# GitHubOfAndrew/TeAMOFlow

Hardware: AMD Instinct MI355X
Metric: train_interactions_per_sec (higher is better)
Workload: dtype f32

## Files before the change

teamoflow_amd/csrc/tmf_common.h:

```cpp
#pragma once
#include <hip/hip_runtime.h>
#include <stdint.h>
#include <stdio.h>

#include <type_traits>

#include "../../include/tmf.h"

namespace tmf {

void set_error(const char* fmt, ...);
int check_launch(const char* what);

#define TMF_REQUIRE(cond, ...)             \
    do {                                   \
        if (!(cond)) {                     \
            tmf::set_error(__VA_ARGS__);   \
            return TMF_E_INVALID;          \
        }                                  \
    } while (0)

inline bool launch_fits(uint64_t blocks, unsigned threads) {
    return blocks > 0 && blocks < (1ull << 31) && blocks * threads < (1ull << 32);
}
// ... 300 lines not shown
    const tmf_f4 t = {v.x, v.y, v.z, v.w};
    __builtin_nontemporal_store(t, reinterpret_cast<tmf_f4*>(p));
}

template <int G, int NV>
__device__ __forceinline__ void store_row(const Frag<NV>& f, float* __restrict__ T, int64_t row, int g) {
    float* p = T + row * (int64_t)(4 * G * NV) + 4 * g;
#pragma unroll
    for (int v = 0; v < NV; ++v) store_f4_nt(p + 4 * G * v, f.v[v]);
}

template <int G, int NV>
__device__ __forceinline__ void store_row(const Frag<NV>& f, __bf16* __restrict__ T, int64_t row, int g) {
    bf16x8* p = reinterpret_cast<bf16x8*>(T + row * (int64_t)(4 * G * NV)) + g;
#pragma unroll
    for (int pv = 0; pv < NV / 2; ++pv) {
        f32x8 w;
        w[0] = f.v[2 * pv].x; w[1] = f.v[2 * pv].y; w[2] = f.v[2 * pv].z; w[3] = f.v[2 * pv].w;
        w[4] = f.v[2 * pv + 1].x; w[5] = f.v[2 * pv + 1].y; w[6] = f.v[2 * pv + 1].z; w[7] = f.v[2 * pv + 1].w;
        __builtin_nontemporal_store(__builtin_convertvector(w, bf16x8), p + G * pv);
    }
}

constexpr bool kNtFin = true;
template <int G, int NV, typename T, bool NT = false>
__device__ __forceinline__ void load_row_f32(Frag<NV>& f, const float* __restrict__ B, int64_t row, int g) {
    const float* p = B + row * (int64_t)(4 * G * NV);
#pragma unroll
    for (int v = 0; v < NV; ++v)
        f.v[v] = NT ? load_f4_nt(p + RowMap<G, NV, T>::off(v, g)) : *reinterpret_cast<const float4*>(p + RowMap<G, NV, T>::off(v, g));
}

template <int G, int NV, typename T>
__device__ __forceinline__ void store_row_f32(const Frag<NV>& f, float* __restrict__ B, int64_t row, int g) {
    float* p = B + row * (int64_t)(4 * G * NV);
#pragma unroll
    for (int v = 0; v < NV; ++v) store_f4_nt(p + RowMap<G, NV, T>::off(v, g), f.v[v]);
}

template <int NV>
__device__ __forceinline__ void zero(Frag<NV>& f) {
#pragma unroll
    for (int v = 0; v < NV; ++v) f.v[v] = make_float4(0.f, 0.f, 0.f, 0.f);
}

template <int NV>
__device__ __forceinline__ float dot_partial(const Frag<NV>& a, const Frag<NV>& b) {
    float s = 0.f;
#pragma unroll
    for (int v = 0; v < NV; ++v) {
        s = fmaf(a.v[v].x, b.v[v].x, s);
        s = fmaf(a.v[v].y, b.v[v].y, s);
        s = fmaf(a.v[v].z, b.v[v].z, s);
        s = fmaf(a.v[v].w, b.v[v].w, s);
    }
    return s;
}

template <int NV>
__device__ __forceinline__ void axpy(Frag<NV>& acc, float w, const Frag<NV>& x) {
#pragma unroll
    for (int v = 0; v < NV; ++v) {
        acc.v[v].x = fmaf(w, x.v[v].x, acc.v[v].x);
        acc.v[v].y = fmaf(w, x.v[v].y, acc.v[v].y);
        acc.v[v].z = fmaf(w, x.v[v].z, acc.v[v].z);
        acc.v[v].w = fmaf(w, x.v[v].w, acc.v[v].w);
    }
}

template <int NV>
__device__ __forceinline__ void add(Frag<NV>& acc, const Frag<NV>& x) {
#pragma unroll
    for (int v = 0; v < NV; ++v) {
        acc.v[v].x += x.v[v].x;
        acc.v[v].y += x.v[v].y;
        acc.v[v].z += x.v[v].z;
        acc.v[v].w += x.v[v].w;
    }
}

__device__ __forceinline__ void wave_lds_sync() {
    __builtin_amdgcn_fence(__ATOMIC_ACQ_REL, "wavefront");
    __builtin_amdgcn_wave_barrier();
}

template <int G>
__device__ __forceinline__ int group_read(int v, int idx) {
    return __shfl(v, (threadIdx.x & 63 & ~(G - 1)) + idx, 64);
}

constexpr int kSyncStride = 16;
__device__ __forceinline__ void step_rendezvous(int* sync, int i, int lag, int n_groups) {
    const int x = blockIdx.x & 7;
    const int mine = (n_groups - x + 7) / 8;
    __hip_atomic_fetch_add(sync + (i * 8 + x) * kSyncStride, 1, __ATOMIC_RELAXED, __HIP_MEMORY_SCOPE_AGENT);
    const int need = i - lag;
    if (need < 0) return;
    for (int spin = 0; spin < 256; ++spin) {
        if (__hip_atomic_load(sync + (need * 8 + x) * kSyncStride, __ATOMIC_RELAXED, __HIP_MEMORY_SCOPE_AGENT) >= mine) return;
        __builtin_amdgcn_s_sleep(8);
    }
}
inline size_t rendezvous_bytes(int64_t launches, int64_t steps) {
    return (size_t)launches * (size_t)steps * 8 * kSyncStride * sizeof(int);
}

#define TMF_DPP_ADD(v, ctrl) \
    ((v) + __int_as_float(__builtin_amdgcn_update_dpp(0, __float_as_int(v), (ctrl), 0xf, 0xf, false)))

template <int G>
__device__ __forceinline__ float group_allsum(float v) {
    if (G >= 2) v = TMF_DPP_ADD(v, 0xB1);
    if (G >= 4) v = TMF_DPP_ADD(v, 0x4E);
    if (G >= 8) v = TMF_DPP_ADD(v, 0x141);
    if (G >= 16) v = TMF_DPP_ADD(v, 0x140);
    if (G >= 32) {
        const auto r = __builtin_amdgcn_permlane16_swap(__float_as_int(v), __float_as_int(v), false, false);
        v = __int_as_float(r[0]) + __int_as_float(r[1]);
    }
    if (G >= 64) {
        const auto r = __builtin_amdgcn_permlane32_swap(__float_as_int(v), __float_as_int(v), false, false);
        v = __int_as_float(r[0]) + __int_as_float(r[1]);
    }
    return v;
}

template <int G>
__device__ __forceinline__ float across_groups_sum(float v) {
#pragma unroll
    for (int off = 32; off >= G; off >>= 1) v += __shfl_xor(v, off, 64);
    return v;
}

template <int G, int NV>
__device__ __forceinline__ void across_groups_sum(Frag<NV>& f) {
#pragma unroll
    for (int v = 0; v < NV; ++v) {
        f.v[v].x = across_groups_sum<G>(f.v[v].x);
        f.v[v].y = across_groups_sum<G>(f.v[v].y);
        f.v[v].z = across_groups_sum<G>(f.v[v].z);
        f.v[v].w = across_groups_sum<G>(f.v[v].w);
    }
}

__device__ __forceinline__ float adam_fresh(float w, float g, const tmf_adam a) {
    const float m = g * a.one_minus_b1;
    const float v = (g * g) * a.one_minus_b2;
    return w - __fdiv_rn(m * a.alpha, __fsqrt_rn(v) + a.eps);
}

template <int NV>
__device__ __forceinline__ void adam_fresh(Frag<NV>& w, const Frag<NV>& g, const tmf_adam a) {
#pragma unroll
    for (int v = 0; v < NV; ++v) {
        w.v[v].x = adam_fresh(w.v[v].x, g.v[v].x, a);
        w.v[v].y = adam_fresh(w.v[v].y, g.v[v].y, a);
        w.v[v].z = adam_fresh(w.v[v].z, g.v[v].z, a);
        w.v[v].w = adam_fresh(w.v[v].w, g.v[v].w, a);
    }
}

template <int G, int NV, typename T>
__device__ __forceinline__ void row_epilogue(const Frag<NV>& g, const T* __restrict__ X_old, void* __restrict__ X_out,
                                             int64_t row, int lane_in_group, int epi, const tmf_adam adam) {
    if (epi == TMF_EPI_GRAD) {
        store_row_f32<G, NV, T>(g, static_cast<float*>(X_out), row, lane_in_group);
// ... 94 lines not shown
```

teamoflow_amd/csrc/tmf_train.hip:

```cpp
#include <stdlib.h>
#include <type_traits>

#include "tmf_common.h"

namespace tmf {

constexpr int kWavesPerBlock = 2;
constexpr int kUnroll = 4;
constexpr int kMseUnroll = 4;
constexpr int64_t kMaxBlocks = ((int64_t)1 << 32) / (64 * kWavesPerBlock) - 1;

struct SegView {
    const int64_t* rowptr;
    const int32_t* seg_row;
    const int32_t* seg_chunk;
    const int32_t* seg_slab;
    int64_t nseg;
    int32_t chunk;
    int32_t row_mod;
    int64_t seg0;
    int xcd_run;
};

struct SegRange { int row; int64_t beg, end; };
// ... 119 lines not shown
                mom[2] += pos ? p : 0.0;
                mom[3] += neg ? p : 0.0;
                mom[4] += pos ? p * p : 0.0;
                mom[5] += neg ? p * p : 0.0;
            } else {
                const double w = pos ? a_pos + b_pos * (p - mu_pos) : a_neg + b_neg * (p - mu_neg);
                axpy<NV>(acc, (pos || neg) ? (float)w : 0.f, y);
            }
        }
    }
    if constexpr (MOMENTS) {
#pragma unroll
        for (int c = 0; c < kKlMoments; ++c) {
#pragma unroll
            for (int off = 32; off >= G; off >>= 1) mom[c] += __shfl_xor(mom[c], off, 64);
        }
        if (lane == 0) {
#pragma unroll
            for (int c = 0; c < kKlMoments; ++c) part[seg * kKlMoments + c] = mom[c];
        }
    } else {
        across_groups_sum<G, NV>(acc);
        if (grp == 0) finish_segment<G, NV, T>(sv, seg, acc, X_old, X_out, slab, row, g, epi, adam);
    }
}

__global__ __launch_bounds__(1024) void k_kl_coeffs(const double* __restrict__ part, int64_t nseg, double* __restrict__ loss_out,
                                                    double* __restrict__ coef) {
    __shared__ double sh[16][kKlMoments];
    const double2* p2 = reinterpret_cast<const double2*>(part);
    const int64_t n2 = 3 * nseg;
    double2 acc[3] = {make_double2(0.0, 0.0), make_double2(0.0, 0.0), make_double2(0.0, 0.0)};
    for (int64_t e0 = threadIdx.x; e0 < n2; e0 += 6 * 1024) {
        double2 v[6];
#pragma unroll
        for (int u = 0; u < 6; ++u) {
            const int64_t e = e0 + (int64_t)u * 1024;
            v[u] = (e < n2) ? p2[e] : make_double2(0.0, 0.0);
        }
#pragma unroll
        for (int u = 0; u < 6; ++u) {
            acc[u % 3].x += v[u].x;
            acc[u % 3].y += v[u].y;
        }
    }
    const int rot = threadIdx.x % 3;
    const double2 m0 = rot == 0 ? acc[0] : rot == 1 ? acc[2] : acc[1];
    const double2 m1 = rot == 0 ? acc[1] : rot == 1 ? acc[0] : acc[2];
    const double2 m2 = rot == 0 ? acc[2] : rot == 1 ? acc[1] : acc[0];
    double s[kKlMoments] = {m0.x, m0.y, m1.x, m1.y, m2.x, m2.y};
#pragma unroll
    for (int c = 0; c < kKlMoments; ++c) {
#pragma unroll
        for (int off = 32; off >= 1; off >>= 1) s[c] += __shfl_xor(s[c], off, 64);
    }
    if ((threadIdx.x & 63) == 0) {
#pragma unroll
        for (int c = 0; c < kKlMoments; ++c) sh[threadIdx.x >> 6][c] = s[c];
    }
    __syncthreads();
    if (threadIdx.x != 0) return;
    double t[kKlMoments];
#pragma unroll
    for (int c = 0; c < kKlMoments; ++c) {
        t[c] = sh[0][c];
        for (int w = 1; w < 16; ++w) t[c] += sh[w][c];
    }
    const double n_pos = t[0], n_neg = t[1];
    const double mu_pos = t[2] / n_pos, mu_neg = t[3] / n_neg;
    const double v_pos = t[4] / n_pos - mu_pos * mu_pos, v_neg = t[5] / n_neg - mu_neg * mu_neg;
    const double sigma = sqrt(v_pos + v_neg), d = mu_pos - mu_neg, z = d / sigma;
    const double phi = exp(-0.5 * z * z) * 0.3989422804014326779;
    loss_out[0] = 0.5 * erfc(z * 0.7071067811865475244);
    coef[0] = -phi / (sigma * n_pos);
    coef[1] = phi * d / (sigma * sigma * sigma * n_pos);
    coef[2] = mu_pos;
    coef[3] = phi / (sigma * n_neg);
    coef[4] = phi * d / (sigma * sigma * sigma * n_neg);
    coef[5] = mu_neg;
}

constexpr int kWsumTile = 512;
constexpr int kWsumUnroll = 4;

template <int G, int NV, typename T>
__global__ __launch_bounds__(64 * kWavesPerBlock) void k_wsum_pass(
    SegView sv, const int32_t* __restrict__ ent_row, const int32_t* __restrict__ ent_w,
    const float* __restrict__ wbuf, const T* __restrict__ Tab, const T* __restrict__ X_old,
    void* __restrict__ X_out, float* __restrict__ slab, int epi, tmf_adam adam) {
    constexpr int NG = 64 / G;
    __shared__ int s_ids[kWavesPerBlock][kWsumTile];
    __shared__ float s_w[kWavesPerBlock][kWsumTile];
    const int lane = threadIdx.x & 63, wave = threadIdx.x >> 6;
    const int64_t seg = sv.seg0 + (int64_t)blockIdx.x * kWavesPerBlock + wave;
    if (seg >= sv.nseg) return;
    const int g = lane & (G - 1), grp = lane / G;
    const int row = sv.seg_row[seg];
    const int64_t rbeg = sv.rowptr[row], rend = sv.rowptr[row + 1];
    const int64_t beg = rbeg + (int64_t)sv.seg_chunk[seg] * sv.chunk;
    const int64_t end = (beg + sv.chunk < rend) ? beg + sv.chunk : rend;
    int* ids = s_ids[wave];
    float* ws = s_w[wave];

    Frag<NV> acc;
    zero<NV>(acc);
    for (int64_t t0 = beg; t0 < end; t0 += kWsumTile) {
        const int cnt = (int)((end - t0 < kWsumTile) ? end - t0 : kWsumTile);
        for (int e = lane; e < cnt; e += 64) {
            ids[e] = ent_row[t0 + e];
            ws[e] = wbuf[ent_w[t0 + e]];
        }
        wave_lds_sync();
        for (int e0 = grp; e0 < cnt; e0 += NG * kUnroll) {
            Raw<NV, T> raw[kUnroll];
            float wc[kUnroll];
#pragma unroll
            for (int t = 0; t < kUnroll; ++t) {
                const int e = e0 + t * NG;
                wc[t] = (e < cnt) ? ws[e] : 0.f;
                if constexpr (std::is_same<T, float>::value) {
                    if (wc[t] != 0.f) load_raw<G, NV>(raw[t], Tab, ids[e], g);
                    else zero_raw<NV>(raw[t]);
                } else {
                    load_raw<G, NV>(raw[t], Tab, ids[wc[t] != 0.f ? e : 0], g);
                }
            }
#pragma unroll
            for (int t = 0; t < kUnroll; ++t) {
                Frag<NV> y;
                to_frag<NV>(y, raw[t]);
                axpy<NV>(acc, wc[t], y);
            }
        }
    }
    across_groups_sum<G, NV>(acc);
    if (grp == 0) finish_segment<G, NV, T>(sv, seg, acc, X_old, X_out, slab, row, g, epi, adam);
}

template <int G, int NV, typename T>
__global__ __launch_bounds__(64 * kWavesPerBlock) void k_wsum_pass_pg(
    SegView sv, const int32_t* __restrict__ ent_row, const int32_t* __restrict__ ent_w,
    const float* __restrict__ wbuf, const T* __restrict__ Tab, const T* __restrict__ X_old,
    void* __restrict__ X_out, float* __restrict__ slab, int epi, tmf_adam adam) {
    constexpr int NG = 64 / G, TILE = kWsumTile / NG;
    __shared__ __attribute__((aligned(16))) int s_ids[kWavesPerBlock][kWsumTile];
    __shared__ __attribute__((aligned(16))) float s_w[kWavesPerBlock][kWsumTile];
    const int lane = threadIdx.x & 63, wave = threadIdx.x >> 6;
    const int g = lane & (G - 1), grp = lane / G;
    int64_t blk = blockIdx.x;
    if (sv.xcd_run > 0) {
        const int64_t super = (int64_t)8 * sv.xcd_run, full = (int64_t)gridDim.x / super * super;
        if (blk < full) {
            const int64_t sc = blk / super, r = blk % super;
            blk = sc * super + (r & 7) * sv.xcd_run + (r >> 3);
        }
    }
    const int64_t seg = sv.seg0 + (blk * kWavesPerBlock + wave) * NG + grp;
    const bool live = seg < sv.nseg;
    const int row = live ? sv.seg_row[seg] : 0;
    int64_t beg = 0, end = 0;
    if (live) {
        const int64_t rbeg = sv.rowptr[row], rend = sv.rowptr[row + 1];
        beg = rbeg + (int64_t)sv.seg_chunk[seg] * sv.chunk;
        end = (beg + sv.chunk < rend) ? beg + sv.chunk : rend;
    }
    int* ids = s_ids[wave] + grp * TILE;
    float* ws = s_w[wave] + grp * TILE;
    Frag<NV> acc;
    zero<NV>(acc);
    for (int64_t t0 = beg; t0 < end; t0 += TILE) {
        const int cnt = (int)((end - t0 < TILE) ? end - t0 : TILE);
        for (int e = g; e < cnt; e += G) {
            ids[e] = ent_row[t0 + e];
            ws[e] = wbuf[ent_w[t0 + e]];
        }
        wave_lds_sync();
        for (int e0 = 0; e0 < cnt; e0 += kWsumUnroll) {
            Raw<NV, T> raw[kWsumUnroll];
            float wc[kWsumUnroll];
#pragma unroll
            for (int t = 0; t < kWsumUnroll; ++t) {
                const int e = e0 + t;
                wc[t] = (e < cnt) ? ws[e] : 0.f;
                if constexpr (std::is_same<T, float>::value) {
                    if (wc[t] != 0.f) load_raw<G, NV>(raw[t], Tab, ids[e], g);
                    else zero_raw<NV>(raw[t]);
                } else {
                    load_raw<G, NV>(raw[t], Tab, ids[wc[t] != 0.f ? e : 0], g);
                }
            }
#pragma unroll
            for (int t = 0; t < kWsumUnroll; ++t) {
                Frag<NV> y;
                to_frag<NV>(y, raw[t]);
                axpy<NV>(acc, wc[t], y);
            }
        }
    }
    if (live) finish_segment<G, NV, T>(sv, seg, acc, X_old, X_out, slab, row, g, epi, adam);
}

constexpr int kRows4Tile = 64;
constexpr int kRows4Unroll2 = 6, kRows4Unroll1 = 4;
constexpr int kRows4Waves = 8;
constexpr int kRows4MinWaves = kRows4Waves / 2;
constexpr int kRows4K2 = 6;

struct VRows {
    const int32_t* item;
    const int32_t* part;
    const int32_t* nparts;
    const int32_t* slot;
    float* slab;
};

template <int G, int NV, typename T, int K, int WAVES>
__global__ __launch_bounds__(64 * WAVES, kRows4MinWaves) void k_wsum_rows4(
    const int64_t* __restrict__ rowptr, int64_t n_rows, int n_blocks, const int32_t* __restrict__ ent_row,
    const int32_t* __restrict__ ent_w, const float* __restrict__ wbuf, const T* __restrict__ Tab, const T* __restrict__ X_old,
    void* __restrict__ X_out, int epi, tmf_adam adam, int64_t row_begin, int64_t row_end, int* __restrict__ sync, int lag,
    VRows vr) {
    static_assert(K + 1 <= G, "the list boundaries of a block live in one register of the lane group");
    constexpr int NG = 64 / G, NGB = NG * WAVES, U = NV >= 2 ? kRows4Unroll2 : kRows4Unroll1;
    __shared__ int s_ids[NGB][kRows4Tile];
    __shared__ float s_w[NGB][kRows4Tile];
    const int tid = threadIdx.x, lane = tid & 63, wave = tid >> 6;
    const int g = lane & (G - 1), gid = wave * NG + lane / G;
    int* ids = s_ids[gid];
    float* ws = s_w[gid];
    const int64_t j0 = row_begin + ((int64_t)blockIdx.x * NGB + gid) * K;
    const int kv = (int)((row_end - j0 < K) ? (row_end > j0 ? row_end - j0 : 0) : K);
    Frag<NV> acc[K];
#pragma unroll
    for (int k = 0; k < K; ++k) zero<NV>(acc[k]);
    const bool balanced = vr.item != nullptr;
    const int64_t vq = j0 + (g < kv ? g : kv);
    const int64_t it = (balanced && kv > 0) ? (int64_t)vr.item[vq] : vq;
    const int pt = (balanced && kv > 0) ? vr.part[vq] : 0, np = (balanced && kv > 0) ? vr.nparts[vq] : 1;
    for (int t = 0; t < n_blocks; ++t) {
        int bnd = 0;
        if (kv > 0) {
            const int64_t lb = rowptr[(int64_t)t * n_rows + it];
            bnd = (int)lb;
            if (np > 1) bnd += (int)(((int64_t)pt * (rowptr[(int64_t)t * n_rows + it + 1] - lb)) / np);
        }
        const int r_beg = group_read<G>(bnd, 0), r_end = group_read<G>(bnd, kv);
        int b[K + 1];
#pragma unroll
        for (int k = 0; k <= K; ++k) b[k] = group_read<G>(bnd, k < kv ? k : kv);
        for (int c0 = r_beg; c0 < r_end; c0 += kRows4Tile) {
            const int cnt = (r_end - c0 < kRows4Tile) ? r_end - c0 : kRows4Tile;
            for (int e = g; e < cnt; e += G) {
                ids[e] = ent_row[c0 + e];
                ws[e] = wbuf[ent_w[c0 + e]];
            }
            wave_lds_sync();
#pragma unroll
            for (int k = 0; k < K; ++k) {
                const int lo = (b[k] > c0 ? b[k] : c0) - c0;
                const int hi = ((b[k + 1] < c0 + cnt) ? b[k + 1] : c0 + cnt) - c0;
                for (int e0 = lo; e0 < hi; e0 += U) {
                    Raw<NV, T> raw[U];
                    float wc[U];
#pragma unroll
                    for (int u = 0; u < U; ++u) {
                        const int e = e0 + u;
                        wc[u] = (e < hi) ? ws[e] : 0.f;
                        load_raw<G, NV>(raw[u], Tab, ids[(wc[u] != 0.f) ? e : lo], g);
                    }
#pragma unroll
                    for (int u = 0; u < U; ++u) {
                        Frag<NV> y;
// ... 461 lines not shown
```

teamoflow_amd/csrc/tmf_wmrb.hip:

```cpp
#include <math.h>
#include <stdlib.h>

#include <type_traits>

#include "tmf_common.h"

namespace tmf {

constexpr int kThreads = 256;
constexpr int kWaves = kThreads / 64;
constexpr int kPosChunk = 512;
constexpr int kUnrollW = 4;
constexpr int kG4Unroll = 4;

__host__ __device__ inline int round4(int x) { return (x + 3) & ~3; }

__host__ __device__ inline int sp_padded(int S) {
    const int nf4 = (S + 3) / 4;
    const int per = ((nf4 + 2 * kWaves - 1) / (2 * kWaves) + 1) & ~1;
    return 4 * 2 * kWaves * per;
}

__device__ __forceinline__ void count_ge0_x4(int& c0, int& c1, float x0, float x1, float x2, float x3) {
    unsigned long long m0, m1, m2, m3;
// ... 230 lines not shown

    across_groups_sum<G, NV>(acc);
#pragma unroll
    for (int off = 32; off >= 1; off >>= 1) {
        lsum += __shfl_xor(lsum, off, 64);
        npos += __shfl_xor(npos, off, 64);
    }
    __syncthreads();
    if (grp == 0) {
#pragma unroll
        for (int v = 0; v < NV; ++v) reinterpret_cast<float4*>(red + wave * LD)[g + G * v] = acc.v[v];
    }
    if (lane == 0) {
        red[kWaves * LD + wave] = lsum;
        red[kWaves * LD + kWaves + wave] = npos;
    }
    __syncthreads();
    if (wave == 0 && grp == 0) {
        Frag<NV> tot;
#pragma unroll
        for (int v = 0; v < NV; ++v) tot.v[v] = reinterpret_cast<const float4*>(red)[g + G * v];
        for (int w = 1; w < kWaves; ++w) {
            Frag<NV> part;
#pragma unroll
            for (int v = 0; v < NV; ++v) part.v[v] = reinterpret_cast<const float4*>(red + w * LD)[g + G * v];
            add<NV>(tot, part);
        }
        row_epilogue<G, NV, T>(tot, U_old, U_out, u, g, epi, adam);
    }
    if (tid == 0) {
        const float* t = red + kWaves * LD;
        if (loss_part) loss_part[u] = (t[0] + t[1]) + (t[2] + t[3]);
        if (pos_part) pos_part[u] = (t[4] + t[5]) + (t[6] + t[7]);
    }
}

template <int G, int NV, typename T>
__global__ __launch_bounds__(kThreads) void k_wmrb_user(
    const int64_t* __restrict__ rowptr, const int32_t* __restrict__ col, const float* __restrict__ val,
    const int32_t* __restrict__ R, int S, float c,
    const T* __restrict__ U_old, const T* __restrict__ V_old, void* __restrict__ U_out, float* __restrict__ delta,
    float* __restrict__ Dg, float* __restrict__ loss_part, float* __restrict__ pos_part, int epi, tmf_adam adam) {
    extern __shared__ __attribute__((aligned(16))) char smem_raw[];
    wmrb_user_body<G, NV, T>(blockIdx.x, smem_raw, rowptr, col, val, R, S, c, U_old, V_old, U_out, delta, Dg, loss_part,
                             pos_part, epi, adam);
}

static size_t wmrb_user_lds(int S, int ld) {
    return sizeof(float) * ((size_t)sp_padded(S) + round4(S) + 4 * kPosChunk + (size_t)round4(S) + 2 * kWaves * 64 +
                            (size_t)kWaves * ld + 2 * kWaves);
}

template <int G, int NV, typename T>
static int launch_wmrb_user(const int64_t* rowptr, const int32_t* col, const float* val, const int32_t* R,
                            int32_t n_users, int32_t S, float c, const T* U_old, const T* V_old,
                            void* U_out, float* delta, float* D, float* loss_part, float* pos_part, int epi,
                            tmf_adam adam, hipStream_t stream) {
    const size_t lds = wmrb_user_lds(S, 4 * G * NV);
    if (lds > 160 * 1024) {
        set_error("wmrb_user_pass: n_samples=%d does not fit LDS (%zu bytes); use the sliced pass (tmf_wmrb_scores3 ...)", S, lds);
        return TMF_E_UNSUPPORTED;
    }
    static LdsGrant grant;
    if (int rc = grant_dynamic_lds(reinterpret_cast<const void*>(&k_wmrb_user<G, NV, T>), lds, grant)) return rc;
    TMF_REQUIRE_LAUNCH(n_users, kThreads, "wmrb_user_pass");
    hipLaunchKernelGGL((k_wmrb_user<G, NV, T>), dim3((unsigned)n_users), dim3(kThreads), lds, stream, rowptr, col,
                       val, R, (int)S, c, U_old, V_old, U_out, delta, D, loss_part, pos_part, epi, adam);
    return check_launch("tmf_wmrb_user_pass");
}

constexpr int kSliceUsers = 16;
constexpr int kLongRange = 48;

template <int G>
struct Stage {
    static constexpr int tile = 8 * G;
};

template <int G>
__device__ __forceinline__ int* slice_stage(char* smem_raw, int gid) {
    return reinterpret_cast<int*>(smem_raw) + gid * 2 * Stage<G>::tile;
}

template <int G, int NV, typename T, bool GRADU>
__device__ __forceinline__ void slice_list(int* ids, float* dst, const int32_t* __restrict__ list, int beg, int end,
                                           const T* __restrict__ V, const Frag<NV>& x, Frag<NV>& acc,
                                           float* __restrict__ out, const float* __restrict__ wts, int g, int safe) {
    constexpr int kStageTile = Stage<G>::tile;
    for (int t0 = beg; t0 < end; t0 += kStageTile) {
        const int cnt = (end - t0 < kStageTile) ? end - t0 : kStageTile;
        for (int e = g; e < cnt; e += G) {
            ids[e] = __builtin_nontemporal_load(list + t0 + e);
            if (GRADU) dst[e] = __builtin_nontemporal_load(wts + t0 + e);
        }
        wave_lds_sync();
        float keep = 0.f;
        for (int e0 = 0; e0 < cnt; e0 += kUnrollW) {
            Raw<NV, T> raw[kUnrollW];
            float d[kUnrollW];
            static_assert(kUnrollW == 4, "vector LDS reads assume four entries per step");
            const int4 id4 = *reinterpret_cast<const int4*>(ids + e0);
            const float4 w4 = GRADU ? *reinterpret_cast<const float4*>(dst + e0) : make_float4(0.f, 0.f, 0.f, 0.f);
            const int idv[4] = {id4.x, id4.y, id4.z, id4.w};
            const float wv[4] = {w4.x, w4.y, w4.z, w4.w};
#pragma unroll
            for (int t = 0; t < kUnrollW; ++t) {
                const int e = e0 + t;
                bool want = e < cnt;
                d[t] = 0.f;
                if (GRADU && want) { d[t] = wv[t]; want = d[t] != 0.f; }
                load_raw<G, NV>(raw[t], V, want ? idv[t] : safe, g);
            }
#pragma unroll
            for (int t = 0; t < kUnrollW; ++t) {
                Frag<NV> y;
                to_frag<NV>(y, raw[t]);
                if (GRADU) {
                    axpy<NV>(acc, d[t], y);
                } else {
                    const int e = e0 + t;
                    const float pr = group_allsum<G>(dot_partial<NV>(x, y));
                    if (g == (e & (G - 1))) keep = pr;
                    if (e < cnt && ((e & (G - 1)) == G - 1 || e == cnt - 1)) {
                        if (g <= (e & (G - 1))) __builtin_nontemporal_store(keep, out + t0 + (e & ~(G - 1)) + g);
                    }
                }
            }
        }
    }
}

template <int NV, typename T>
__device__ __forceinline__ void slice_scores_lean(int* ids, const int32_t* __restrict__ list, int beg, int end, const T* __restrict__ V,
                                                  const Raw<NV, T>& x, float* __restrict__ out, int g, int lane, int safe) {
    constexpr int G = 32, kStageTile = Stage<G>::tile;
    const uint32_t loff = 16u * (uint32_t)g;
    const int my_entry = Reduce4x32::entry_of_lane(lane);
    const int my_step = lane & 7, my_slot = 4 * my_step + my_entry;
    for (int t0 = beg; t0 < end; t0 += kStageTile) {
        const int cnt = (end - t0 < kStageTile) ? end - t0 : kStageTile;
        const int cnt4 = (cnt + 3) & ~3;
        for (int e = g; e < cnt4; e += G) ids[e] = e < cnt ? __builtin_nontemporal_load(list + t0 + e) : safe;
        wave_lds_sync();
        float keep = 0.f;
        for (int e0 = 0; e0 < cnt4; e0 += 4) {
            const int4 id4 = *reinterpret_cast<const int4*>(ids + e0);
            Raw<NV, T> y[4];
            load_raw32<G, NV>(y[0], V, (uint32_t)id4.x, loff);
            load_raw32<G, NV>(y[1], V, (uint32_t)id4.y, loff);
            load_raw32<G, NV>(y[2], V, (uint32_t)id4.z, loff);
            load_raw32<G, NV>(y[3], V, (uint32_t)id4.w, loff);
            float pr[4];
#pragma unroll
            for (int t = 0; t < 4; ++t) pr[t] = dot_raw<NV>(x, y[t]);
            const float sc = Reduce4x32::run(pr, lane);
            const int step = (e0 >> 2) & 7;
            keep = (step == my_step) ? sc : keep;
            if (step == 7 || e0 + 4 >= cnt4) {
                const int at = (e0 & ~31) + my_slot;
                if (at < cnt) __builtin_nontemporal_store(keep, out + t0 + at);
            }
        }
    }
}

struct SliceLists {
    const int32_t* R;
    const int32_t* off;
    const int64_t* rowptr;
    const int32_t* col;
    const int32_t* poff;
    int n_slices, S;
    int64_t n_users, n_groups;
    int upg;
    int sl0, nsl;
    int item_base;
    int xcd;
    int lean;
};

__device__ __forceinline__ bool slice_of_block(const SliceLists& a, int64_t b, int64_t& sl, int64_t& grp) {
    if (!a.xcd) {
        sl = a.sl0 + b / a.n_groups;
        grp = b % a.n_groups;
        return true;
    }
    const int64_t x = b & 7, j = b >> 3;
    sl = a.sl0 + 8 * (j / a.n_groups) + x;
    grp = j % a.n_groups;
    return sl < a.sl0 + a.nsl;
}

template <int G, int NV, typename T>
__device__ __forceinline__ const T* window_base(const T* V, int item_base) {
    return V - (int64_t)item_base * (4 * G * NV);
}

template <int G, int NV, typename T, int WAVES>
__global__ __launch_bounds__(64 * WAVES) void k_wmrb_scores3(SliceLists a, const T* __restrict__ U, const T* __restrict__ V,
                                                           float* __restrict__ sp, float* __restrict__ p) {
    extern __shared__ __attribute__((aligned(16))) char smem_raw[];
    constexpr int NG = 64 / G, NGB = NG * WAVES;
    const int tid = threadIdx.x, lane = tid & 63, wave = tid >> 6;
    const int g = lane & (G - 1), gid = wave * NG + lane / G;
    int* ids = slice_stage<G>(smem_raw, gid);
    float* dst = reinterpret_cast<float*>(ids + Stage<G>::tile);
    int64_t sl, grp;
    if (!slice_of_block(a, blockIdx.x, sl, grp)) return;
    const int64_t ubeg = grp * a.upg;
    const int64_t uend = (ubeg + a.upg < a.n_users) ? ubeg + a.upg : a.n_users;
    V = window_base<G, NV, T>(V, a.item_base);
    if constexpr (G == 32 && sizeof(Raw<NV, T>) <= 16) {
        if (a.lean) {
            for (int64_t u = ubeg + gid; u < uend; u += NGB) {
                const int64_t o = u * (a.n_slices + 1) + sl;
                const int nb = a.off[o], ne = a.off[o + 1], pb = a.poff[o], pe = a.poff[o + 1];
                if (nb == ne && pb == pe) continue;
                Raw<NV, T> x;
                {
                    const char* xp = reinterpret_cast<const char*>(U) + u * (int64_t)RowBytes<G, NV, T>::value + 16 * g;
                    if constexpr (std::is_same<T, float>::value) {
#pragma unroll
                        for (int v = 0; v < NV; ++v) x.v[v] = load_f4_nt(reinterpret_cast<const float*>(xp + 16 * G * v));
                    } else {
#pragma unroll
                        for (int pv = 0; pv < NV / 2; ++pv) x.v[pv] = __builtin_nontemporal_load(reinterpret_cast<const bf16x8*>(xp + 16 * G * pv));
                    }
                }
                slice_scores_lean<NV, T>(ids, a.R + u * (int64_t)a.S, nb, ne, V, x, sp + u * (int64_t)a.S, g, lane, a.item_base);
                const int64_t rb = a.rowptr[u];
                slice_scores_lean<NV, T>(ids, a.col + rb, pb, pe, V, x, p + rb, g, lane, a.item_base);
            }
            return;
        }
    }
    for (int64_t u = ubeg + gid; u < uend; u += NGB) {
        const int64_t o = u * (a.n_slices + 1) + sl;
        const int nb = a.off[o], ne = a.off[o + 1], pb = a.poff[o], pe = a.poff[o + 1];
        if (nb == ne && pb == pe) continue;
        Frag<NV> x, none;
        load_row_nt<G, NV>(x, U, u, g);
        slice_list<G, NV, T, false>(ids, dst, a.R + u * (int64_t)a.S, nb, ne, V, x, none, sp + u * (int64_t)a.S, nullptr, g,
                                    a.item_base);
        const int64_t rb = a.rowptr[u];
        slice_list<G, NV, T, false>(ids, dst, a.col + rb, pb, pe, V, x, none, p + rb, nullptr, g, a.item_base);
    }
}

template <int G, int NV, typename T, int WAVES>
__global__ __launch_bounds__(64 * WAVES) void k_wmrb_gradu3(SliceLists a, const T* __restrict__ V, const float* __restrict__ D,
                                                          const float* __restrict__ delta, float* __restrict__ part,
                                                          int slice_first, int accumulate) {
    extern __shared__ __attribute__((aligned(16))) char smem_raw[];
    constexpr int NG = 64 / G, NGB = NG * WAVES;
    const int tid = threadIdx.x, lane = tid & 63, wave = tid >> 6;
    const int g = lane & (G - 1), gid = wave * NG + lane / G;
    int* ids = slice_stage<G>(smem_raw, gid);
    float* dst = reinterpret_cast<float*>(ids + Stage<G>::tile);
    int64_t sl, grp, layer = 0;
    if (slice_first < 0) {
        if (!slice_of_block(a, blockIdx.x, sl, grp)) return;
    } else if (accumulate >= 3) {
        layer = blockIdx.x & 7;
        sl = slice_first + layer;
        grp = blockIdx.x >> 3;
        if (sl >= a.sl0 + a.nsl) return;
        accumulate -= 2;
    } else {
        sl = slice_first;
        grp = blockIdx.x;
    }
    V = window_base<G, NV, T>(V, a.item_base);
    const int64_t ubeg = grp * a.upg;
    const int64_t uend = (ubeg + a.upg < a.n_users) ? ubeg + a.upg : a.n_users;
    for (int64_t u = ubeg + gid; u < uend; u += NGB) {
        const int64_t o = u * (a.n_slices + 1) + sl;
        const int nb = a.off[o], ne = a.off[o + 1], pb = a.poff[o], pe = a.poff[o + 1];
        Frag<NV> acc, none;
        zero<NV>(acc);
        const int64_t us = u * (int64_t)a.S, rb = a.rowptr[u];
        slice_list<G, NV, T, true>(ids, dst, a.R + us, nb, ne, V, none, acc, nullptr, D + us, g, a.item_base);
        slice_list<G, NV, T, true>(ids, dst, a.col + rb, pb, pe, V, none, acc, nullptr, delta + rb, g, a.item_base);
        if (accumulate == 0) {
            store_row_f32<G, NV, T>(acc, part, sl * a.n_users + u, g);
        } else {
            const int64_t prow = layer * a.n_users + u;
            if (accumulate == 2) {
                Frag<NV> prev;
                load_row_f32<G, NV, T>(prev, part, prow, g);
                add<NV>(prev, acc);
                acc = prev;
            }
            store_row_f32<G, NV, T>(acc, part, prow, g);
        }
    }
}

template <int G>
struct Stage4 {
    static constexpr int cap = G < 16 ? G : 16;
};

template <int G, int NV, typename T, int K, int WAVES>
__global__ __launch_bounds__(64 * WAVES, WAVES / 2) void k_wmrb_gradu4(
    SliceLists a, const T* __restrict__ V, const float* __restrict__ D,
                                                          const float* __restrict__ delta, const T* __restrict__ U_old,
                                                          void* __restrict__ U_out, int epi, tmf_adam adam, int64_t user_begin,
                                                          int64_t user_end, int* __restrict__ sync, int lag) {
    extern __shared__ __attribute__((aligned(16))) char smem_raw[];
    constexpr int NG = 64 / G, NGB = NG * WAVES, CAP = Stage4<G>::cap, WIN = G - 1, UG = (CAP >= 8) ? kG4Unroll : kUnrollW;
    const int tid = threadIdx.x, lane = tid & 63, wave = tid >> 6;
    const int g = lane & (G - 1), gid = wave * NG + lane / G;
    int* stage = reinterpret_cast<int*>(smem_raw) + gid * (2 * K * 2 * CAP);
    V = window_base<G, NV, T>(V, a.item_base);
    const int64_t u0 = user_begin + ((int64_t)blockIdx.x * NGB + gid) * K;
    const int sl_end = a.sl0 + a.nsl;
    Frag<NV> acc[K];
    int us[K], rb[K];
    bool live[K];
    int ocn[K], ocp[K];
    int c_tot[K];
#pragma unroll
    for (int k = 0; k < K; ++k) {
        zero<NV>(acc[k]);
        live[k] = u0 + k < user_end;
        const int64_t u = live[k] ? u0 + k : user_begin;
        us[k] = (int)(u * (int64_t)a.S);
        rb[k] = (int)a.rowptr[u];
    }
    int base = a.sl0;
    auto refill = [&](int b) {
        base = b;
#pragma unroll
        for (int k = 0; k < K; ++k) {
            const int64_t u = live[k] ? u0 + k : user_begin;
            const int64_t o = u * (a.n_slices + 1) + ((b + g <= a.n_slices) ? b + g : a.n_slices);
            ocn[k] = a.off[o];
            ocp[k] = a.poff[o];
        }
    };
    int n_tot[K], n_id[K];
    float n_w[K];
    auto fetch = [&](int sl) {
#pragma unroll
        for (int k = 0; k < K; ++k) {
            const int nb = group_read<G>(ocn[k], sl - base), ne = group_read<G>(ocn[k], sl + 1 - base);
            const int pb = group_read<G>(ocp[k], sl - base), pe = group_read<G>(ocp[k], sl + 1 - base);
            const int cn = live[k] ? ne - nb : 0;
            n_tot[k] = live[k] ? cn + (pe - pb) : 0;
            const bool neg = g < cn, any = g < n_tot[k] && g < CAP;
            const int at = neg ? us[k] + nb + g : rb[k] + pb + (g - cn);
            n_id[k] = any ? (neg ? a.R : a.col)[at] : a.item_base;
            n_w[k] = any ? (neg ? D : delta)[at] : 0.f;
        }
    };
    auto commit = [&](int buf) {
#pragma unroll
        for (int k = 0; k < K; ++k) {
            int* ids = stage + (buf * K + k) * 2 * CAP;
            if (g < CAP) {
                ids[g] = n_id[k];
                reinterpret_cast<float*>(ids + CAP)[g] = n_w[k];
            }
            c_tot[k] = n_tot[k];
        }
// ... 766 lines not shown
```

Before: 1.148 billion.

## Compact nonzero-weight entries via ballot before gathering embedding rows

```diff
diff --git a/teamoflow_amd/csrc/tmf_common.h b/teamoflow_amd/csrc/tmf_common.h
--- a/teamoflow_amd/csrc/tmf_common.h
+++ b/teamoflow_amd/csrc/tmf_common.h
@@ -406,6 +406,33 @@
 __device__ __forceinline__ void wave_lds_sync() {
     __builtin_amdgcn_fence(__ATOMIC_ACQ_REL, "wavefront");
     __builtin_amdgcn_wave_barrier();
+}
+
+template <int G, int STEP>
+__device__ __forceinline__ void stage_nonzero(int* ids, float* ws, int& n, int id, float w, int g) {
+    const bool nz = w != 0.f;
+    uint64_t b = __builtin_amdgcn_ballot_w64(nz);
+    if constexpr (G < 64) b = (b >> (threadIdx.x & 63 & ~(G - 1))) & ((1ull << G) - 1);
+    if (nz) {
+        const int at = n + __popcll(b & ((1ull << g) - 1));
+        ids[at] = id;
+        ws[at] = w;
+        if ((b >> g) == 1) {
+#pragma unroll
+            for (int k = 1; k < STEP; ++k) {
+                if ((at & (STEP - 1)) + k < STEP) {
+                    ids[at + k] = id;
+                    ws[at + k] = 0.f;
+                }
+            }
+        }
+    }
+    n += __popcll(b);
+}
+
+template <int STEP>
+__device__ __forceinline__ int staged_steps(int n) {
+    return (n + STEP - 1) / STEP * STEP;
 }
 
 template <int G>
diff --git a/teamoflow_amd/csrc/tmf_train.hip b/teamoflow_amd/csrc/tmf_train.hip
--- a/teamoflow_amd/csrc/tmf_train.hip
+++ b/teamoflow_amd/csrc/tmf_train.hip
@@ -225,6 +225,7 @@
 
 constexpr int kWsumTile = 512;
 constexpr int kWsumUnroll = 4;
+constexpr int kWsumRounds = 4;
 
 template <int G, int NV, typename T>
 __global__ __launch_bounds__(64 * kWavesPerBlock) void k_wsum_pass(
@@ -245,28 +246,54 @@
     int* ids = s_ids[wave];
     float* ws = s_w[wave];
 
+    constexpr int SUB = kWsumTile / NG;
+    constexpr uint64_t kClass0 = NG == 64 ? 1ull : ~0ull / ((1ull << (NG & 63)) - 1);
+    static_assert(SUB % kUnroll == 0, "a class's slots hold its padded count");
+    const int cls = lane & (NG - 1);
+    const uint64_t in_cls = kClass0 << cls, in_grp = kClass0 << grp, below = (1ull << lane) - 1;
     Frag<NV> acc;
     zero<NV>(acc);
     for (int64_t t0 = beg; t0 < end; t0 += kWsumTile) {
         const int cnt = (int)((end - t0 < kWsumTile) ? end - t0 : kWsumTile);
-        for (int e = lane; e < cnt; e += 64) {
-            ids[e] = ent_row[t0 + e];
-            ws[e] = wbuf[ent_w[t0 + e]];
-        }
+        int n_cls = 0, n = 0;
+        for (int e0 = 0; e0 < cnt; e0 += 64) {
+            const int e = e0 + lane;
+            int id = 0;
+            float w = 0.f;
+            if (e < cnt) {
+                id = ent_row[t0 + e];
+                w = wbuf[ent_w[t0 + e]];
+            }
+            const bool nz = w != 0.f;
+            const uint64_t b = __builtin_amdgcn_ballot_w64(nz);
+            if (nz) {
+                const int at = cls * SUB + n_cls + __popcll(b & in_cls & below);
+                ids[at] = id;
+                ws[at] = w;
+                if (((b & in_cls) >> lane) == 1) {
+#pragma unroll
+                    for (int k = 1; k < kUnroll; ++k) {
+                        if ((at & (kUnroll - 1)) + k < kUnroll) {
+                            ids[at + k] = id;
+                            ws[at + k] = 0.f;
+                        }
+                    }
+                }
+            }
+            n_cls += __popcll(b & in_cls);
+            n += __popcll(b & in_grp);
+        }
+        const int* idg = ids + grp * SUB;
+        const float* wsg = ws + grp * SUB;
+        n = staged_steps<kUnroll>(n);
         wave_lds_sync();
-        for (int e0 = grp; e0 < cnt; e0 += NG * kUnroll) {
+        for (int e0 = 0; e0 < n; e0 += kUnroll) {
             Raw<NV, T> raw[kUnroll];
             float wc[kUnroll];
 #pragma unroll
             for (int t = 0; t < kUnroll; ++t) {
-                const int e = e0 + t * NG;
-                wc[t] = (e < cnt) ? ws[e] : 0.f;
-                if constexpr (std::is_same<T, float>::value) {
-                    if (wc[t] != 0.f) load_raw<G, NV>(raw[t], Tab, ids[e], g);
-                    else zero_raw<NV>(raw[t]);
-                } else {
-                    load_raw<G, NV>(raw[t], Tab, ids[wc[t] != 0.f ? e : 0], g);
-                }
+                wc[t] = wsg[e0 + t];
+                load_raw<G, NV>(raw[t], Tab, idg[e0 + t], g);
             }
 #pragma unroll
             for (int t = 0; t < kUnroll; ++t) {
@@ -311,26 +338,36 @@
     float* ws = s_w[wave] + grp * TILE;
     Frag<NV> acc;
     zero<NV>(acc);
+    static_assert(TILE % kWsumUnroll == 0, "the tile buffers hold the padded count");
     for (int64_t t0 = beg; t0 < end; t0 += TILE) {
         const int cnt = (int)((end - t0 < TILE) ? end - t0 : TILE);
-        for (int e = g; e < cnt; e += G) {
-            ids[e] = ent_row[t0 + e];
-            ws[e] = wbuf[ent_w[t0 + e]];
-        }
+        int n = 0;
+        for (int e0 = 0; e0 < cnt; e0 += kWsumRounds * G) {
+            int id[kWsumRounds], iw[kWsumRounds];
+            float w[kWsumRounds];
+#pragma unroll
+            for (int k = 0; k < kWsumRounds; ++k) {
+                const int e = e0 + k * G + g;
+                id[k] = iw[k] = -1;
+                if (e < cnt) {
+                    id[k] = ent_row[t0 + e];
+                    iw[k] = ent_w[t0 + e];
+                }
+            }
+#pragma unroll
+            for (int k = 0; k < kWsumRounds; ++k) w[k] = iw[k] >= 0 ? wbuf[iw[k]] : 0.f;
+#pragma unroll
+            for (int k = 0; k < kWsumRounds; ++k) stage_nonzero<G, kWsumUnroll>(ids, ws, n, id[k], w[k], g);
+        }
+        n = staged_steps<kWsumUnroll>(n);
         wave_lds_sync();
-        for (int e0 = 0; e0 < cnt; e0 += kWsumUnroll) {
+        for (int e0 = 0; e0 < n; e0 += kWsumUnroll) {
             Raw<NV, T> raw[kWsumUnroll];
             float wc[kWsumUnroll];
 #pragma unroll
             for (int t = 0; t < kWsumUnroll; ++t) {
-                const int e = e0 + t;
-                wc[t] = (e < cnt) ? ws[e] : 0.f;
-                if constexpr (std::is_same<T, float>::value) {
-                    if (wc[t] != 0.f) load_raw<G, NV>(raw[t], Tab, ids[e], g);
-                    else zero_raw<NV>(raw[t]);
-                } else {
-                    load_raw<G, NV>(raw[t], Tab, ids[wc[t] != 0.f ? e : 0], g);
-                }
+                wc[t] = ws[e0 + t];
+                load_raw<G, NV>(raw[t], Tab, ids[e0 + t], g);
             }
 #pragma unroll
             for (int t = 0; t < kWsumUnroll; ++t) {
diff --git a/teamoflow_amd/csrc/tmf_wmrb.hip b/teamoflow_amd/csrc/tmf_wmrb.hip
--- a/teamoflow_amd/csrc/tmf_wmrb.hip
+++ b/teamoflow_amd/csrc/tmf_wmrb.hip
@@ -336,51 +336,86 @@
     return reinterpret_cast<int*>(smem_raw) + gid * 2 * Stage<G>::tile;
 }
 
-template <int G, int NV, typename T, bool GRADU>
-__device__ __forceinline__ void slice_list(int* ids, float* dst, const int32_t* __restrict__ list, int beg, int end,
-                                           const T* __restrict__ V, const Frag<NV>& x, Frag<NV>& acc,
-                                           float* __restrict__ out, const float* __restrict__ wts, int g, int safe) {
+template <int G, int NV, typename T>
+__device__ __forceinline__ void slice_list(int* ids, const int32_t* __restrict__ list, int beg, int end, const T* __restrict__ V,
+                                           const Frag<NV>& x, float* __restrict__ out, int g, int safe) {
     constexpr int kStageTile = Stage<G>::tile;
+    static_assert(kUnrollW == 4, "vector LDS reads assume four entries per step");
     for (int t0 = beg; t0 < end; t0 += kStageTile) {
         const int cnt = (end - t0 < kStageTile) ? end - t0 : kStageTile;
-        for (int e = g; e < cnt; e += G) {
-            ids[e] = __builtin_nontemporal_load(list + t0 + e);
-            if (GRADU) dst[e] = __builtin_nontemporal_load(wts + t0 + e);
-        }
+        for (int e = g; e < cnt; e += G) ids[e] = __builtin_nontemporal_load(list + t0 + e);
         wave_lds_sync();
         float keep = 0.f;
         for (int e0 = 0; e0 < cnt; e0 += kUnrollW) {
             Raw<NV, T> raw[kUnrollW];
-            float d[kUnrollW];
-            static_assert(kUnrollW == 4, "vector LDS reads assume four entries per step");
             const int4 id4 = *reinterpret_cast<const int4*>(ids + e0);
-            const float4 w4 = GRADU ? *reinterpret_cast<const float4*>(dst + e0) : make_float4(0.f, 0.f, 0.f, 0.f);
             const int idv[4] = {id4.x, id4.y, id4.z, id4.w};
-            const float wv[4] = {w4.x, w4.y, w4.z, w4.w};
-#pragma unroll
-            for (int t = 0; t < kUnrollW; ++t) {
-                const int e = e0 + t;
-                bool want = e < cnt;
-                d[t] = 0.f;
-                if (GRADU && want) { d[t] = wv[t]; want = d[t] != 0.f; }
-                load_raw<G, NV>(raw[t], V, want ? idv[t] : safe, g);
-            }
+#pragma unroll
+            for (int t = 0; t < kUnrollW; ++t)
+                load_raw<G, NV>(raw[t], V, e0 + t < cnt ? idv[t] : safe, g);
 #pragma unroll
             for (int t = 0; t < kUnrollW; ++t) {
                 Frag<NV> y;
                 to_frag<NV>(y, raw[t]);
-                if (GRADU) {
-                    axpy<NV>(acc, d[t], y);
-                } else {
-                    const int e = e0 + t;
-                    const float pr = group_allsum<G>(dot_partial<NV>(x, y));
-                    if (g == (e & (G - 1))) keep = pr;
-                    if (e < cnt && ((e & (G - 1)) == G - 1 || e == cnt - 1)) {
-                        if (g <= (e & (G - 1))) __builtin_nontemporal_store(keep, out + t0 + (e & ~(G - 1)) + g);
-                    }
+                const int e = e0 + t;
+                const float pr = group_allsum<G>(dot_partial<NV>(x, y));
+                if (g == (e & (G - 1))) keep = pr;
+                if (e < cnt && ((e & (G - 1)) == G - 1 || e == cnt - 1)) {
+                    if (g <= (e & (G - 1))) __builtin_nontemporal_store(keep, out + t0 + (e & ~(G - 1)) + g);
                 }
             }
         }
+    }
+}
+
+constexpr int kStageRounds = 4;
+
+template <int G, int NV, typename T>
+__device__ __forceinline__ void gather_staged(const int* ids, const float* ws, int n, const T* __restrict__ V, Frag<NV>& acc, int g) {
+    static_assert(kUnrollW == 4, "vector LDS reads assume four entries per step");
+    wave_lds_sync();
+    for (int e0 = 0; e0 < n; e0 += kUnrollW) {
+        Raw<NV, T> raw[kUnrollW];
+        const int4 id4 = *reinterpret_cast<const int4*>(ids + e0);
+        const float4 w4 = *reinterpret_cast<const float4*>(ws + e0);
+        const int idv[4] = {id4.x, id4.y, id4.z, id4.w};
+        const float wv[4] = {w4.x, w4.y, w4.z, w4.w};
+#pragma unroll
+        for (int t = 0; t < kUnrollW; ++t) load_raw<G, NV>(raw[t], V, idv[t], g);
+#pragma unroll
+        for (int t = 0; t < kUnrollW; ++t) {
+            Frag<NV> y;
+            to_frag<NV>(y, raw[t]);
+            axpy<NV>(acc, wv[t], y);
+        }
+    }
+}
+
+template <int G, int NV, typename T>
+__device__ __forceinline__ void slice_append(int* ids, float* ws, int& n, const int32_t* __restrict__ list,
+                                            const float* __restrict__ wts, int beg, int end, const T* __restrict__ V,
+                                            Frag<NV>& acc, int g) {
+    constexpr int kStageTile = Stage<G>::tile;
+    static_assert(kStageRounds * 2 <= 8, "a tile of 8 G entries holds two loads of rounds");
+    for (int e0 = beg; e0 < end; e0 += kStageRounds * G) {
+        if (n > kStageTile - kStageRounds * G) {
+            gather_staged<G, NV, T>(ids, ws, staged_steps<kUnrollW>(n), V, acc, g);
+            n = 0;
+        }
+        int id[kStageRounds];
+        float w[kStageRounds];
+#pragma unroll
+        for (int k = 0; k < kStageRounds; ++k) {
+            const int e = e0 + k * G + g;
+            id[k] = 0;
+            w[k] = 0.f;
+            if (e < end) {
+                id[k] = __builtin_nontemporal_load(list + e);
+                w[k] = __builtin_nontemporal_load(wts + e);
+            }
+        }
+#pragma unroll
+        for (int k = 0; k < kStageRounds; ++k) stage_nonzero<G, kUnrollW>(ids, ws, n, id[k], w[k], g);
     }
 }
 
@@ -458,7 +493,6 @@
     const int tid = threadIdx.x, lane = tid & 63, wave = tid >> 6;
     const int g = lane & (G - 1), gid = wave * NG + lane / G;
     int* ids = slice_stage<G>(smem_raw, gid);
-    float* dst = reinterpret_cast<float*>(ids + Stage<G>::tile);
     int64_t sl, grp;
     if (!slice_of_block(a, blockIdx.x, sl, grp)) return;
     const int64_t ubeg = grp * a.upg;
@@ -492,12 +526,11 @@
         const int64_t o = u * (a.n_slices + 1) + sl;
         const int nb = a.off[o], ne = a.off[o + 1], pb = a.poff[o], pe = a.poff[o + 1];
         if (nb == ne && pb == pe) continue;
-        Frag<NV> x, none;
+        Frag<NV> x;
         load_row_nt<G, NV>(x, U, u, g);
-        slice_list<G, NV, T, false>(ids, dst, a.R + u * (int64_t)a.S, nb, ne, V, x, none, sp + u * (int64_t)a.S, nullptr, g,
-                                    a.item_base);
+        slice_list<G, NV, T>(ids, a.R + u * (int64_t)a.S, nb, ne, V, x, sp + u * (int64_t)a.S, g, a.item_base);
         const int64_t rb = a.rowptr[u];
-        slice_list<G, NV, T, false>(ids, dst, a.col + rb, pb, pe, V, x, none, p + rb, nullptr, g, a.item_base);
+        slice_list<G, NV, T>(ids, a.col + rb, pb, pe, V, x, p + rb, g, a.item_base);
     }
 }
 
@@ -530,11 +563,13 @@
     for (int64_t u = ubeg + gid; u < uend; u += NGB) {
         const int64_t o = u * (a.n_slices + 1) + sl;
         const int nb = a.off[o], ne = a.off[o + 1], pb = a.poff[o], pe = a.poff[o + 1];
-        Frag<NV> acc, none;
+        Frag<NV> acc;
         zero<NV>(acc);
         const int64_t us = u * (int64_t)a.S, rb = a.rowptr[u];
-        slice_list<G, NV, T, true>(ids, dst, a.R + us, nb, ne, V, none, acc, nullptr, D + us, g, a.item_base);
-        slice_list<G, NV, T, true>(ids, dst, a.col + rb, pb, pe, V, none, acc, nullptr, delta + rb, g, a.item_base);
+        int n = 0;
+        slice_append<G, NV, T>(ids, dst, n, a.R + us, D + us, nb, ne, V, acc, g);
+        slice_append<G, NV, T>(ids, dst, n, a.col + rb, delta + rb, pb, pe, V, acc, g);
+        gather_staged<G, NV, T>(ids, dst, staged_steps<kUnrollW>(n), V, acc, g);
         if (accumulate == 0) {
             store_row_f32<G, NV, T>(acc, part, sl * a.n_users + u, g);
         } else {
```

Result: faster. 1.172 billion, median of 6 (+2.0%).
